# phbgomes22/FastFourierConvolution

Measured on AMD Instinct MI355X. Metric: FFC-generator fwd images/sec @ B=256 64×64×3; % HBM roofline; max |Δ| vs ref, higher is better.
Workload: dtype f32; 1 GPU; FFCGenerator(nz=100,nc=3,ngf=64) forward 64x64x3; global_batch=256, per_gpu_batch=256, bn_mode=train, spectral_mix=fp32, hipgraph=True, parallelism=dp1

## Files before the change

### fastfourierconvolution_amd/_plan.py

```python
from __future__ import annotations

from dataclasses import dataclass, field

import os

import numpy as np

CONVQ_TCMAX = int(os.environ.get("FFC_CONVQ_TCMAX", "0"))

BK = 16
MPAD = 128
TILE_CFGS = {0: (128, 128, 2), 1: (64, 128, 2), 2: (32, 256, 4)}
PAD_ENTRY = (15, 0, 0, 0)


@dataclass(frozen=True)
class Seg:
    kind: str
    C: int
    IH: int
    IW: int
    k: int = 1
    s: int = 1
    p: int = 0
# ... 202 lines not shown
    OH: int
    OW: int
    Sy: int
    Sx: int
    segs: tuple
    mults: list
    cpad: list
    org: list
    prc: list
    vec4: list
    rowlen: list
    phases: list
    ktab: np.ndarray
    taptab: np.ndarray
    a_size: int
    cfg: int
    NS: int
    TR: int
    TC: int
    nrb: int
    ncb: int
    cc: list = field(default_factory=list)
    q: bool = False
    mt: int = 1
    direct: list = field(default_factory=list)
    qstride: list = field(default_factory=list)
    ksplit: int = 1

    @property
    def Mpad(self):
        return -(-self.M // MPAD) * MPAD

    @property
    def npb(self):
        return -(-self.B // self.NS) * self.nrb * self.ncb


PATCH_MAX_UNITS = 8 * 256


def patch_units_per_row(PC: int, vec4: bool, aligned: bool = False) -> int:
    if not vec4:
        return PC
    return -(-PC // 4) if aligned else (PC + 6) // 4


def plan_patch_job(B: int, M: int, segs, cfg: int | None = None):
    segs = tuple(segs)
    if any(sg.pool or sg.gate for sg in segs):
        return None
    base = plan_job(B, M, segs)
    NP = base.Sy * base.Sx
    if NP not in (1, 4) or len(base.phases) != NP:
        return None
    if cfg is None:
        cfg = 0 if NP == 4 else 2
    np_, ntw = PATCH_CFGS[cfg]
    if np_ != NP:
        return None
    npix = (4 // NP) * ntw * 32
    PHm = max(ph.PH for ph in base.phases)
    PWm = max(ph.PW for ph in base.phases)
    TC = min(PWm, npix)
    TR = min(PHm, max(1, npix // TC))
    NS = max(1, min(B, npix // (TR * TC)))
    nrb, ncb = -(-PHm // TR), -(-PWm // TC)
    taps = []
    cc = [PATCH_CC] * len(segs)
    for ph in base.phases:
        row = []
        for si, sg in enumerate(segs):
            ty = _taps(sg, base.Sy, ph.py, sg.IH, ph.PH)
            tx = _taps(sg, base.Sx, ph.px, sg.IW, ph.PW)
            if NP == 1 and len(ty) == len(tx) == 3 and (sg.kind == "conv" or (sg.kind == "convT" and sg.s == 1)):
                ty, tx = sorted(ty, key=lambda t: t[1]), sorted(tx, key=lambda t: t[1])
                if any(b[1] - a[1] != 1 for a, b in zip(ty, ty[1:])) or any(b[1] - a[1] != 1 for a, b in zip(tx, tx[1:])):
                    return None
                ty = ty + [(-1, ty[-1][1] + 1)]
                tx = tx + [(-1, tx[-1][1] + 1)]
            T = len(ty) * len(tx)
            if T == 16 and NP == 1 and len(ty) == len(tx) == 4:
                cc[si] = 4
            elif T and 4 % T:
                return None
            row.append((ty, tx))
        taps.append(row)
    cpad = [-(-sg.C // cc[si]) * cc[si] for si, sg in enumerate(segs)]
    org, prc, vec4, rowlen = [], [], [], []
    for si, sg in enumerate(segs):
        oys = [o for row in taps for (k, o) in row[si][0]]
        oxs = [o for row in taps for (k, o) in row[si][1]]
        if not oys or not oxs:
            oys, oxs = [0], [0]
        my_, mx_ = base.mults[si]
        oy0, ox0 = min(oys), min(oxs)
        PR = (TR - 1) * my_ + (max(oys) - oy0) + 1
        PC = (TC - 1) * mx_ + (max(oxs) - ox0) + 1
        v4 = sg.IW % 4 == 0
        al = ox0 % 4 == 0 and (TC * mx_) % 4 == 0
        if NS * cc[si] * PR * patch_units_per_row(PC, v4, al) > PATCH_MAX_UNITS:
            return None
        vec4.append(v4)
        rowlen.append(4 * patch_units_per_row(PC, True, al) if v4 else PC)
        org.append((oy0, ox0))
        prc.append((PR, PC))
    phases, ktab, taptab = [], [], []
    a_total = 0
    Mpad = -(-M // MPAD) * MPAD
    for pi, ph in enumerate(base.phases):
        d = dict(py=ph.py, px=ph.px, PH=ph.PH, PW=ph.PW, T=[], kseg=[], tap_base=[], tap_h=[])
        k = 0
        kt_off = len(ktab)
        for si, sg in enumerate(segs):
            ty, tx = taps[pi][si]
            T = len(ty) * len(tx)
            d["T"].append(T)
            d["kseg"].append(k)
            d["tap_base"].append(len(taptab))
            PR, PC = prc[si]
            base_t = len(taptab)
            for (ky, oy) in ty:
                for (kx, ox) in tx:
                    taptab.append(((oy - org[si][0]) << 16) | (ox - org[si][1]))
            th = 0
            if T == 16:
                dyx = [(t >> 16, t & 0xFFFF) for t in taptab[base_t:]]
                hy, hx = dyx[8][0] - dyx[0][0], dyx[8][1] - dyx[0][1]
                if hx < 0 or any((dyx[j + 8][0] - dyx[j][0], dyx[j + 8][1] - dyx[j][1]) != (hy, hx)
                                 for j in range(8)):
                    return None
                th = (hy << 16) | hx
            d["tap_h"].append(th)
            for ch in range(cpad[si]):
                for (ky, oy) in ty:
                    for (kx, ox) in tx:
                        ktab.append((si | (ch << 4), oy, ox, ky | (kx << 16))
                                    if ch < sg.C and ky >= 0 and kx >= 0 else PAD_ENTRY)
            k += cpad[si] * T
        if k == 0:
            return None
        d["Kpad"] = k
        d["K"] = k
        d["kt_off"] = kt_off
        d["a_off"] = a_total
        a_total += Mpad * k
        phases.append(d)
    return PatchPlan(B, M, base.OH, base.OW, base.Sy, base.Sx, segs, base.mults, cpad, org, prc, vec4, rowlen, phases,
                     np.asarray(ktab, dtype=np.int32).reshape(-1, 4), np.asarray(taptab or [0], dtype=np.int32),
                     a_total, cfg, NS, TR, TC, nrb, ncb, cc)


CONVQ_CFGS = {0: (1, 4), 1: (1, 2), 2: (2, 2), 3: (1, 1)}
CONVQ_MAX_UNITS = 256
CONVQ_LDS_BUDGET = 150 * 1024


def convq_strides(NS, TR, TC, PR, PC, pad=True):
    if not pad:
        return PC, PR * PC
    qr = PC + ((TC - PC) % 16)
    qs = PR * qr + ((TR * TC - PR * qr) % 16)
    return qr, qs


def convq_lds_bytes(NS, strides):
    return 3 * (((max(NS * qs for _, qs in strides) * 96 + 255) // 256) * 256 + 256)


def plan_convq_job(B: int, M: int, segs, cfg: int):
    segs = tuple(segs)
    if any(sg.pool or sg.gate for sg in segs):
        return None
    base = plan_job(B, M, segs)
    if (base.Sy, base.Sx) != (2, 2) or len(base.phases) != 4:
        return None
    mt, ntw = CONVQ_CFGS[cfg]
    npix = 32 * ntw
    PHm = max(ph.PH for ph in base.phases)
    PWm = max(ph.PW for ph in base.phases)
    TC = min(PWm, npix)
    if CONVQ_TCMAX >= 4 and TC > CONVQ_TCMAX:
        TC = CONVQ_TCMAX
    TR = min(PHm, max(1, npix // TC))
    NS = max(1, min(B, npix // (TR * TC)))
    nrb, ncb = -(-PHm // TR), -(-PWm // TC)
    direct = [sg.kind == "pw" for sg in segs]
    taps = []
    for ph in base.phases:
        row = []
        for si, sg in enumerate(segs):
            ty = _taps(sg, base.Sy, ph.py, sg.IH, ph.PH)
            tx = _taps(sg, base.Sx, ph.px, sg.IW, ph.PW)
            T = len(ty) * len(tx)
            if (direct[si] and T not in (0, 1)) or T > 4:
                return None
            row.append((ty, tx))
        taps.append(row)
    cpad = [-(-sg.C // 16) * 16 for sg in segs]
    org, prc = [], []
    for si, sg in enumerate(segs):
        my_, mx_ = base.mults[si]
        if direct[si]:
            if (my_, mx_) != (2, 2):
                return None
            org.append((0, 0))
            prc.append((1, 1))
            continue
        oys = [o for row in taps for (k, o) in row[si][0]] or [0]
        oxs = [o for row in taps for (k, o) in row[si][1]] or [0]
        oy0, ox0 = min(oys), min(oxs)
        PR = (TR - 1) * my_ + (max(oys) - oy0) + 1
        PC = (TC - 1) * mx_ + (max(oxs) - ox0) + 1
        if sg.IW % 4:
            return None
        PC = 4 * patch_units_per_row(PC, True, False)
        if 2 * NS * PR * (PC // 4) > CONVQ_MAX_UNITS:
            return None
        org.append((oy0, ox0))
        prc.append((PR, PC))
    staged = [prc[si] for si in range(len(segs)) if not direct[si]]
    pad = bool(staged) and convq_lds_bytes(NS, [convq_strides(NS, TR, TC, PR, PC) for PR, PC in staged]) \
        <= CONVQ_LDS_BUDGET
    if os.environ.get("FFC_CONVQ_PAD") == "0":
        pad = False
    qstride = [convq_strides(NS, TR, TC, PR, PC, pad) for (PR, PC) in prc]
    if staged and convq_lds_bytes(NS, [qstride[si] for si in range(len(segs)) if not direct[si]]) > 160 * 1024:
        return None
    if any(not direct[si] and B * sg.C * sg.IH * sg.IW * 4 >= 0x7FFFFFFF for si, sg in enumerate(segs)):
        return None
    phases, ktab, taptab = [], [], []
    a_total = 0
    Mpad = -(-M // MPAD) * MPAD
    for pi, ph in enumerate(base.phases):
        d = dict(py=ph.py, px=ph.px, PH=ph.PH, PW=ph.PW, T=[], kseg=[], tap_base=[], tap_h=[])
        k = 0
        kt_off = len(ktab)
        for si, sg in enumerate(segs):
            ty, tx = taps[pi][si]
            T = len(ty) * len(tx)
            d["T"].append(T)
            d["kseg"].append(k)
            d["tap_base"].append(len(taptab))
            d["tap_h"].append(0)
            tl = [(ky, oy, kx, ox) for (ky, oy) in ty for (kx, ox) in tx]
            TT = 1 if direct[si] else 4
            d["T"][-1] = TT
            for t in range(TT):
                taptab.append(((tl[t][1] - org[si][0]) << 16) | (tl[t][3] - org[si][1]) if t < T else 0)
            for c0 in range(0, cpad[si], 16):
                for t in range(TT):
                    for ch in range(c0, c0 + 16):
                        if t < T and ch < sg.C:
                            ky, oy, kx, ox = tl[t]
                            ktab.append((si | (ch << 4), oy, ox, ky | (kx << 16)))
                        else:
                            ktab.append(PAD_ENTRY)
            k += cpad[si] * TT
        if k == 0:
            return None
        d["Kpad"] = k
        d["K"] = k
        d["kt_off"] = kt_off
        d["a_off"] = a_total
        a_total += Mpad * k
        phases.append(d)
    return PatchPlan(B, M, base.OH, base.OW, base.Sy, base.Sx, segs, base.mults, cpad, org, prc,
                     [not d for d in direct], [pc for (_, pc) in prc], phases,
                     np.asarray(ktab, dtype=np.int32).reshape(-1, 4), np.asarray(taptab or [0], dtype=np.int32),
                     a_total, cfg, NS, TR, TC, nrb, ncb, [16] * len(segs), True, mt, direct, qstride)


CONVQ_SPLIT_FIXED = 17500.0


def convq_chunks(q) -> int:
    return sum(c // 16 for c in q.cpad)


def convq_cost(q, ksplit: int = 1) -> float:
    wgs = q.npb * (-(-q.M // (32 * q.mt))) * ksplit
    mt, ntw = CONVQ_CFGS[q.cfg]
    slots = 256 * (2 if (mt, ntw) == (1, 1) else 1)
    per_wg = -(-convq_chunks(q) // ksplit) * (768.0 * mt * ntw + 5500.0)
    return -(-wgs // slots) * (per_wg + (CONVQ_SPLIT_FIXED if ksplit > 1 else 0.0))


_TUNED = None


def job_signature(B, M, segs) -> tuple:
    return (int(B), int(M), tuple((sg.kind, sg.C, sg.IH, sg.IW, sg.k, sg.s, sg.p, sg.d, sg.op, sg.pool, sg.gate)
                                  for sg in segs))


def convq_tuned():
    global _TUNED
    if _TUNED is None:
        import json
        jobs, groups = {}, {}
        path = os.environ.get("FFC_CONVQ_TUNED", os.path.join(os.path.dirname(os.path.abspath(__file__)),
                                                               "convq_tuned.json"))
        if path and os.path.exists(path):
            with open(path) as f:
                for e in json.load(f)["entries"]:
                    sigs = tuple(sorted((B, M, tuple(tuple(sg) for sg in segs)) for B, M, segs in e["jobs"]))
                    groups[sigs] = (int(e["cfg"]), int(e["ksplit"]))
                    for sg in sigs:
                        jobs[sg] = int(e["cfg"])
        _TUNED = (jobs, groups)
    return _TUNED


def pick_convq_ksplit(q) -> int:
    return pick_convq_ksplit_group([q])


def pick_convq_ksplit_group(plans) -> int:
    cmin = min(convq_chunks(q) for q in plans)
    force = os.environ.get("FFC_CONVQ_KSPLIT")
    if force is not None:
        return max(1, min(8, int(force), cmin))
    tuned = convq_tuned()[1].get(tuple(sorted(job_signature(q.B, q.M, q.segs) for q in plans)))
    if tuned is not None and tuned[0] == plans[0].cfg:
        return max(1, min(tuned[1], cmin))
    ks = [k for k in (1, 2, 4, 8) if k == 1 or cmin >= 4 * k]
    return min(ks, key=lambda k: (sum(convq_cost(q, k) for q in plans), k))


def convq_slot_tiles(tiles) -> np.ndarray:
    first = tiles[(tiles[:, 3] & 7) == 0]
    out = np.zeros((first.shape[0], 4), dtype=np.int32)
    out[first[:, 3] >> 3, :3] = first[:, :3]
    return out


def pick_convq_cfg(B, M, segs):
    force = os.environ.get("FFC_CONVQ_CFG")
    tuned = convq_tuned()[0].get(job_signature(B, M, segs))
    if os.environ.get("FFC_CONVQ_TUNED_LOG"):
        import sys
        print(f"[convq] tuned cfg {'hit' if tuned is not None else 'miss'}: {job_signature(B, M, segs)}",
              file=sys.stderr)
    if force is not None:
        cands = [int(force)]
    elif tuned is not None:
        cands = [tuned]
    else:
        cands = ([0, 2] if M >= 64 else [0]) + [1, 3]
    plans = [q for q in (plan_convq_job(B, M, segs, c) for c in cands) if q is not None]
    for q in plans:
        q.ksplit = pick_convq_ksplit(q)
    return min(plans, key=lambda q: convq_cost(q, q.ksplit)) if plans else None


def pick_patch_cfg(B, M, segs, min_blocks=512):
    force = os.environ.get("FFC_PATCH_CFG4")
    if force is not None:
        q = plan_patch_job(B, M, segs, int(force))
        if q is not None:
            return q
    p = plan_patch_job(B, M, segs)
    if p is None:
        return plan_patch_job(B, M, segs, 1) or plan_patch_job(B, M, segs, 3)
    if p.cfg == 0:
        blocks = p.npb * (-(-M // 32))
        if blocks < min_blocks:
            q = plan_patch_job(B, M, segs, 1)
            if q is not None:
                return q
# ... 32 lines not shown
```

### fastfourierconvolution_amd/csrc/convq_kernels.hip

```cpp
#include "ffc_internal.h"

#include <algorithm>
#include <cstdlib>
#include <map>
#include <mutex>
#include <string>
#include <tuple>

namespace {

constexpr int QTHREADS = 512;
#ifndef FFC_CONVQ_WPE
#define FFC_CONVQ_WPE
#endif
#ifndef FFC_CONVQ_SLOTS
#define FFC_CONVQ_SLOTS 2
#endif
constexpr int QSLOTS = FFC_CONVQ_SLOTS;
static_assert(QSLOTS >= 2 && QSLOTS <= 6, "convq staging slots");

struct ConvQArgs {
    ffc_convp_job jobs[2];
    const int4* tiles;
    int ebuf;
// ... 119 lines not shown
        if (cl == 0 && m < E.M) stp[m] = make_float4(cnt, mean, m2, 0.0f);
    }
}

template <int MT, int NTW>
__device__ __forceinline__ void convq_epilogue(const ffc_convp_job& J, int wave, int lane, int pb, int m0,
                                               floatx16 (&acc)[MT][NTW]) {
    const QGeom<NTW> g = q_geometry<NTW>(J, wave, lane, pb);
    const ffc_convp_phase& P = J.ph[wave];
    const QEpi E = q_epi(J);
    const int py = P.py, px = P.px;
    const int h = lane >> 5, cl = lane & 31;
    const size_t plane = (size_t)E.OH * E.OW;
    long long obase[NTW];
#pragma unroll
    for (int nt = 0; nt < NTW; ++nt)
        obase[nt] = (long long)(g.b0 + g.pns[nt]) * E.M * (long long)plane +
                    ((g.r0 + g.pr_[nt]) * 2 + py) * E.OW + ((g.c0 + g.pc_[nt]) * 2 + px);
    bool allv = m0 + 32 * MT <= E.M;
#pragma unroll
    for (int nt = 0; nt < NTW; ++nt) allv = allv && g.pv[nt];
    const bool full = __builtin_amdgcn_ballot_w64(allv) == ~0ull;
    unsigned voff[NTW];
#pragma unroll
    for (int nt = 0; nt < NTW; ++nt) {
        voff[nt] = ((unsigned)g.pns[nt] * (unsigned)E.M * (unsigned)plane + (unsigned)(4 * h) * (unsigned)plane +
                    (unsigned)(((g.r0 + g.pr_[nt]) * 2 + py) * E.OW + ((g.c0 + g.pc_[nt]) * 2 + px))) * 4u;
        asm volatile("" : "+v"(voff[nt]));
    }
#pragma unroll
    for (int mt = 0; mt < MT; ++mt) {
        floatx16 (&tacc)[NTW] = acc[mt];
        const int mbase = m0 + 32 * mt + 4 * h;
        if (E.bias || E.addend) {
#pragma unroll
            for (int r = 0; r < 16; ++r) {
                const int m = mbase + (r & 3) + 8 * (r >> 2);
                if (m >= E.M) continue;
                const float bv = E.bias ? E.bias[m] : 0.0f;
#pragma unroll
                for (int nt = 0; nt < NTW; ++nt) {
                    float v = tacc[nt][r] + bv;
                    if (E.addend && g.pv[nt]) v += E.addend[obase[nt] + (long long)m * plane];
                    tacc[nt][r] = v;
                }
            }
        }
        if (E.stats) q_stats<NTW>(E, wave, cl, pb, mbase, g.pv, tacc);
        if (full) {
#pragma unroll
            for (int r = 0; r < 16; ++r) {
                float* sb = E.out + ((size_t)g.b0 * E.M + m0 + 32 * mt + (r & 3) + 8 * (r >> 2)) * plane;
#pragma unroll
                for (int nt = 0; nt < NTW; ++nt) {
                    *reinterpret_cast<float*>(reinterpret_cast<char*>(sb) + voff[nt]) = q_act(tacc[nt][r], E.slope);
                }
            }
            continue;
        }
#pragma unroll
        for (int r = 0; r < 16; ++r) {
            const int m = mbase + (r & 3) + 8 * (r >> 2);
            if (m < E.M) {
#pragma unroll
                for (int nt = 0; nt < NTW; ++nt)
                    if (g.pv[nt]) E.out[obase[nt] + (long long)m * plane] = q_act(tacc[nt][r], E.slope);
            }
        }
    }
}

typedef float floatx2 __attribute__((ext_vector_type(2)));
template <int PX>
struct StageVec {
    float v[PX];
};
template <int PX>
__device__ __forceinline__ StageVec<PX> stage_ld(__amdgpu_buffer_rsrc_t rs, int voff, int soff) {
    StageVec<PX> r;
    if constexpr (PX == 4) {
        const floatx4 q = __builtin_bit_cast(floatx4, __builtin_amdgcn_raw_buffer_load_b128(rs, voff, soff, 0));
        r.v[0] = q[0]; r.v[1] = q[1]; r.v[2] = q[2]; r.v[3] = q[3];
    } else if constexpr (PX == 2) {
        const floatx2 q = __builtin_bit_cast(floatx2, __builtin_amdgcn_raw_buffer_load_b64(rs, voff, soff, 0));
        r.v[0] = q[0]; r.v[1] = q[1];
    } else {
        r.v[0] = __builtin_bit_cast(float, __builtin_amdgcn_raw_buffer_load_b32(rs, voff, soff, 0));
    }
    return r;
}

template <int MT, int NTW, int SL = QSLOTS, int PX = 4>
__device__ __forceinline__ void convq_tile(const ConvQArgs& args, const int tix, char* lds) {
    static_assert(SL >= 2 && SL <= 6, "convq staging slots");
    static_assert(PX == 1 || PX == 2 || PX == 4, "pixels per staging unit");
    const int tid = threadIdx.x, lane = tid & 63;
    const int wave_id = __builtin_amdgcn_readfirstlane(tid >> 6);
    const bool stager = wave_id >= 4;
    const int wave = wave_id & 3;
    const int stid = tid - 256;
    const int h = lane >> 5, cl = lane & 31;
    const int4 tile = args.tiles[tix];
    const int ji = __builtin_amdgcn_readfirstlane(tile.x);
    const int m0 = __builtin_amdgcn_readfirstlane(tile.y);
    const int pb = __builtin_amdgcn_readfirstlane(tile.z);
    const int tw = __builtin_amdgcn_readfirstlane(tile.w);
    const int ks = tw & 7, slot = tw >> 3;
    const int nsplit = args.ksplit;
    const ffc_convp_job& J = args.jobs[ji];
    const ffc_convp_phase& P = J.ph[wave];
    const int ebuf = args.ebuf;

    const int NS = J.NS, TR = J.TR, TC = J.TC;
    const int bs = pb / (J.nrb * J.ncb);
    const int prem = pb - bs * J.nrb * J.ncb;
    const int rb = prem / J.ncb, cb = prem - rb * J.ncb;
    const int b0 = bs * NS, r0 = rb * TR, c0 = cb * TC;
    const int TRC = TR * TC;
    const int nseg = J.nseg;


    floatx16 acc[MT][NTW];
#pragma unroll
    for (int mt = 0; mt < MT; ++mt)
#pragma unroll
        for (int nt = 0; nt < NTW; ++nt)
#pragma unroll
            for (int r = 0; r < 16; ++r) acc[mt][nt][r] = 0.0f;

#ifdef FFC_TRACE_Q
    const unsigned long long tq_rt0 = __builtin_amdgcn_s_memrealtime();
    unsigned long long tq_0, tq_a, tq_b, tq_c, tq_d, tq_bar = 0, tq_A = 0, tq_mf = 0;
    QSTAMP(tq_0);
#endif
    const int ksteps = P.Kpad >> 4;
    const uint16_t* __restrict__ Afrag = J.A3 + 3 * P.a_off + (size_t)(m0 >> 5) * ksteps * 1536 + lane * 8;
    auto load_A = [&](int k, Split3 (&a)[MT]) {
#pragma unroll
        for (int mt = 0; mt < MT; ++mt) {
            const uint16_t* f = Afrag + ((size_t)mt * ksteps + (k >> 4)) * 1536;
            a[mt].hi = __builtin_bit_cast(bf16x8, *reinterpret_cast<const u32x4*>(f));
            a[mt].mid = __builtin_bit_cast(bf16x8, *reinterpret_cast<const u32x4*>(f + 512));
            a[mt].lo = __builtin_bit_cast(bf16x8, *reinterpret_cast<const u32x4*>(f + 1024));
        }
    };

    struct {
        __amdgpu_buffer_rsrc_t rs;
        unsigned voff;
        unsigned cstride;
        int C, Cpad, cfull;
        int hu8;
        int wb;
    } st;
    auto stage_setup = [&](int s) {
        const ffc_convp_seg& S = J.seg[s];
        const int IHW = S.IH * S.IW;
        st.rs = ffc::buf_rsrc(S.x, (unsigned long long)J.B * S.C * IHW * 4);
        st.C = S.C;
        st.Cpad = S.Cpad;
        st.cfull = (S.C & 15) == 0;
        st.cstride = (unsigned)IHW * 4u;
        const int PR = S.PR, G = S.PC / PX, QR = S.qrow, QS = S.qsample;
        const int ngrp = NS * PR * G;
        const int nunits = 2 * ngrp;
        const int iy0 = r0 * S.mult_y + S.org_y;
        const int xa = (c0 * S.mult_x + S.org_x) & ~3;
        const int n = stid;
        const int hu = n >= ngrp ? 1 : 0;
        const int q = n - hu * ngrp;
        const int g = q % G, q1 = q / G;
        const int pr = q1 % PR, ns = q1 / PR;
        const int b = b0 + ns, iy = iy0 + pr, ix = xa + PX * g;
        const bool ok = n < nunits && b < J.B && (unsigned)iy < (unsigned)S.IH && (unsigned)ix < (unsigned)S.IW;
        st.voff = ok ? (unsigned)(((b * S.C + 8 * hu) * IHW + iy * S.IW + ix) * 4) : ffc::OOB;
        st.hu8 = 8 * hu;
        st.wb = n < nunits ? ((hu * NS + ns) * QS + pr * QR + PX * g) * 48 : -1;
    };
    auto stage_load = [&](StageVec<PX> (&sv)[8], int ch0) {
        const unsigned sbase = (unsigned)ch0 * st.cstride;
#pragma unroll
        for (int j = 0; j < 8; ++j) {
            const unsigned vo = (st.cfull || ch0 + st.hu8 + j < st.C) ? st.voff : ffc::OOB;
            sv[j] = stage_ld<PX>(st.rs, (int)vo, (int)(sbase + (unsigned)j * st.cstride));
        }
    };
    auto stage_store = [&](const StageVec<PX> (&sv)[8], int wb, char* buf) {
        if (wb >= 0) {
#pragma unroll
            for (int e = 0; e < PX; ++e) {
                float v8[8];
#pragma unroll
                for (int j = 0; j < 8; ++j) v8[j] = sv[j].v[e];
                const Split3 sp = split3(v8);
                u32x4* d = reinterpret_cast<u32x4*>(buf + wb + 48 * e);
                d[0] = __builtin_bit_cast(u32x4, sp.hi);
                d[1] = __builtin_bit_cast(u32x4, sp.mid);
                d[2] = __builtin_bit_cast(u32x4, sp.lo);
            }
        }
    };

    int kseg = 0, cpad = 0;
    int fb[NTW];
    int tb[4];
    auto geom = [&](int s, int (&fbo)[NTW], int (&tbo)[4]) {
        const ffc_convp_seg& S = J.seg[s];
        const QGeom<NTW> g = q_geometry<NTW>(J, wave, lane, pb);
        const int QR = S.qrow, QS = S.qsample, nimg = NS * QS;
        const int ix0 = c0 * S.mult_x + S.org_x, xoff = ix0 - (ix0 & ~3);
#pragma unroll
        for (int nt = 0; nt < NTW; ++nt)
            fbo[nt] = (h * nimg + g.pns[nt] * QS + g.pr_[nt] * S.mult_y * QR + g.pc_[nt] * S.mult_x + xoff) * 48;
#pragma unroll
        for (int t = 0; t < 4; ++t) {
            const int tt = P.tap[s][t];
            tbo[t] = ((tt >> 16) * QR + (tt & 0xFFFF)) * 48;
        }
    };
    auto compute_setup = [&](int s) {
        kseg = P.kseg[s];
        cpad = J.seg[s].Cpad;
        geom(s, fb, tb);
    };

    int nstaged = 0, ndirect = 0;
    for (int s = 0; s < nseg; ++s) {
        if (J.seg[s].direct) ndirect += J.seg[s].Cpad >> 4;
        else nstaged += J.seg[s].Cpad >> 4;
    }
    const int ntot = nstaged + ndirect;
    const int lo = ntot * ks / nsplit, hi = ntot * (ks + 1) / nsplit;
    const int slo = min(lo, nstaged), nst = min(hi, nstaged) - slo;
    const int dlo = max(lo, nstaged) - nstaged, dhi = max(hi, nstaged) - nstaged;

    const int npad = (nst + SL - 1) / SL * SL;
    if (nst > 0) {
        int ss = 0;
        while (J.seg[ss].direct) ++ss;
        int c0k = slo;
        while (c0k >= (J.seg[ss].Cpad >> 4)) {
            c0k -= J.seg[ss].Cpad >> 4;
            do { ++ss; } while (J.seg[ss].direct);
        }
        int cs = ss, sch = 16 * c0k, cch = 16 * c0k;
        if (stager) {
#ifdef FFC_TRACE_Q
            unsigned long long q0, qa, qb, ql = 0, qs = 0, qw = 0, qi = 0;
            QSTAMP(q0);
#endif
            StageVec<PX> sv[SL][8];
            int wbs[SL];
            stage_setup(ss);
            int ic = 0;
            auto issue = [&](StageVec<PX> (&dst)[8], int& wb) {
                const bool live = ss < nseg && ic < nst;
                ++ic;
                stage_load(dst, live ? sch : 0);
                wb = live ? st.wb : -1;
                if (live) {
                    sch += 16;
                    if (sch >= st.Cpad) {
                        do { ++ss; } while (ss < nseg && J.seg[ss].direct);
                        sch = 0;
                        if (ss < nseg) stage_setup(ss);
                    }
                }
            };
            auto store_timed = [&](const StageVec<PX> (&src)[8], int wb, char* buf) {
#ifdef FFC_TRACE_Q
                QSTAMP(qa);
                float chk = src[0].v[0] + src[7].v[PX - 1];
                asm volatile("" ::"v"(chk));
                QSTAMP(qb);
                ql += qb - qa;
                stage_store(src, wb, buf);
                QSTAMP(qa);
                qs += qa - qb;
#else
                stage_store(src, wb, buf);
#endif
            };
            auto bar = [&]() {
#ifdef FFC_TRACE_Q
                QSTAMP(qa);
#endif
#ifndef FFC_QPROBE_NOBAR
                __syncthreads();
#endif
#ifdef FFC_TRACE_Q
                QSTAMP(qb);
                qw += qb - qa;
#endif
            };
#pragma unroll
            for (int u = 0; u < SL; ++u) issue(sv[u], wbs[u]);
            store_timed(sv[0], wbs[0], lds);
            issue(sv[0], wbs[0]);
            store_timed(sv[1 % SL], wbs[1 % SL], lds + ebuf);
            bar();
            int wbuf = 2;
            for (int c0 = 1; c0 <= npad; c0 += SL) {
#pragma unroll
                for (int u = 0; u < SL; ++u) {
#ifndef FFC_QPROBE_NOSTAGE
#ifdef FFC_TRACE_Q
                    QSTAMP(qa);
#endif
                    issue(sv[(1 + u) % SL], wbs[(1 + u) % SL]);
#ifdef FFC_TRACE_Q
                    QSTAMP(qb);
                    qi += qb - qa;
#endif
                    store_timed(sv[(2 + u) % SL], wbs[(2 + u) % SL], lds + wbuf * ebuf);
#endif
                    wbuf = wbuf == 2 ? 0 : wbuf + 1;
                    bar();
                }
            }
#ifdef FFC_TRACE_Q
            QSTAMP(qa);
            if (tid == 256) {
                unsigned long long* tr = g_ffc_trace_q + 16 * tix;
                tr[9] = ql;
                tr[10] = qs;
                tr[11] = qw;
                tr[12] = qa - q0;
                tr[13] = nst;
                tr[14] = qi;
            }
#endif
            return;
        }
        Split3 a[4][MT];
        compute_setup(cs);
        int pf[NTW];
#pragma unroll
        for (int nt = 0; nt < NTW; ++nt) pf[nt] = fb[nt] + tb[0];
#pragma unroll
        for (int t = 0; t < 4; ++t) load_A(kseg + cch * 4 + 16 * t, a[t]);
        u32x4 bq[2][NTW][3];
        auto read_frag = [&](const char* base, const int (&off)[NTW], int add, u32x4 (&dst)[NTW][3]) {
#pragma unroll
            for (int nt = 0; nt < NTW; ++nt) {
                const char* p1 = base + off[nt] + add;
                dst[nt][0] = lds_read16(p1, 0);
                dst[nt][1] = lds_read16(p1, 16);
                dst[nt][2] = lds_read16(p1, 32);
            }
        };
#ifdef FFC_TRACE_Q
        QSTAMP(tq_a);
#endif
        __syncthreads();
#ifdef FFC_TRACE_Q
        QSTAMP(tq_b);
        tq_bar += tq_b - tq_a;
#endif
        read_frag(lds, pf, 0, bq[0]);
        int rbuf = 0;
        for (int ci = 0; ci < nst; ++ci) {
#ifdef FFC_TRACE_Q
            QSTAMP(tq_a);
#endif
            const bool more = ci + 1 < nst;
            const int nbuf = rbuf == 2 ? 0 : rbuf + 1;
            const char* cur = lds + rbuf * ebuf;
            const char* nxt = lds + nbuf * ebuf;
            int cn = cs, chn = cch + 16;
            const bool segchg = more && chn >= cpad;
            int kn;
            if (segchg) {
                do { ++cn; } while (J.seg[cn].direct);
                chn = 0;
                kn = P.kseg[cn];
                int fbn[NTW], tbn[4];
                geom(cn, fbn, tbn);
#pragma unroll
                for (int nt = 0; nt < NTW; ++nt) pf[nt] = fbn[nt] + tbn[0];
            } else {
                kn = kseg + (more ? chn : cch) * 4;
            }
            __builtin_amdgcn_sched_barrier(0);
#ifdef FFC_TRACE_Q
            QSTAMP(tq_b);
            tq_A += tq_b - tq_a;
#endif
#ifndef FFC_QPROBE_NOMFMA
#pragma unroll
            for (int t = 0; t < 4; ++t) {
                if (t + 1 < 4) read_frag(cur, fb, tb[t + 1], bq[(t + 1) & 1]);
                else read_frag(nxt, pf, 0, bq[0]);
#pragma unroll
                for (int nt = 0; nt < NTW; ++nt) {
                    Split3 b;
                    b.hi = __builtin_bit_cast(bf16x8, bq[t & 1][nt][0]);
                    b.mid = __builtin_bit_cast(bf16x8, bq[t & 1][nt][1]);
                    b.lo = __builtin_bit_cast(bf16x8, bq[t & 1][nt][2]);
#pragma unroll
                    for (int mt = 0; mt < MT; ++mt) acc[mt][nt] = mfma_split3(a[t][mt], b, acc[mt][nt]);
                }
#ifndef FFC_QPROBE_NOA
                load_A(kn + 16 * t, a[t]);
#endif
                __builtin_amdgcn_sched_group_barrier(0x100, 3 * NTW, 0);
                __builtin_amdgcn_sched_group_barrier(0x8, 6 * NTW * MT, 0);
                __builtin_amdgcn_sched_group_barrier(0x20, 3 * MT, 0);
                __builtin_amdgcn_sched_barrier(0);
            }
#endif
#ifdef FFC_TRACE_Q
            QSTAMP(tq_a);
            tq_mf += tq_a - tq_b;
#endif
            if (segchg) {
                cs = cn;
                cch = 0;
                compute_setup(cs);
            } else {
                cch += 16;
            }
            rbuf = nbuf;
#ifdef FFC_TRACE_Q
            QSTAMP(tq_a);
#endif
#ifndef FFC_QPROBE_NOBAR
            __syncthreads();
#endif
#ifdef FFC_TRACE_Q
            QSTAMP(tq_b);
            tq_bar += tq_b - tq_a;
#endif
        }
#ifndef FFC_QPROBE_NOBAR
        for (int ci = nst; ci < npad; ++ci) __syncthreads();
#endif
    }
#ifdef FFC_TRACE_Q
    QSTAMP(tq_c);
#endif
    if (stager) return;

    int dbase = 0;
    for (int s = 0; s < nseg; ++s) {
        const ffc_convp_seg& S = J.seg[s];
        if (!S.direct) continue;
        const int nch = S.Cpad >> 4;
        const int c_lo = max(dlo - dbase, 0), c_hi = min(dhi - dbase, nch);
        dbase += nch;
        if (c_lo >= c_hi) continue;
        const int IHW = S.IH * S.IW;
        const QGeom<NTW> g = q_geometry<NTW>(J, wave, lane, pb);
        const bool* pv = g.pv;
        const float* xp[NTW];
#pragma unroll
        for (int nt = 0; nt < NTW; ++nt) {
            const int oy = (r0 + g.pr_[nt]) * J.Sy + P.py, ox = (c0 + g.pc_[nt]) * J.Sx + P.px;
            const int b = pv[nt] ? b0 + g.pns[nt] : 0;
            xp[nt] = S.x + ((long long)b * S.C + 8 * h) * IHW + (pv[nt] ? oy * S.IW + ox : 0);
        }
        for (int ch0 = 16 * c_lo; ch0 < 16 * c_hi; ch0 += 16) {
            Split3 a[MT];
            load_A(P.kseg[s] + ch0, a);
            float bv[NTW][8];
#pragma unroll
            for (int nt = 0; nt < NTW; ++nt)
#pragma unroll
// ... 3 lines not shown
                    bv[nt][j] = ok ? v : 0.0f;
                }
#pragma unroll
            for (int nt = 0; nt < NTW; ++nt) {
                const Split3 b = split3(bv[nt]);
#pragma unroll
                for (int mt = 0; mt < MT; ++mt) acc[mt][nt] = mfma_split3(a[mt], b, acc[mt][nt]);
            }
        }
    }

#ifdef FFC_QPROBE_NOEPI
    if (acc[0][0][0] != 1234.5f) return;
#endif
    if (nsplit > 1) {
        store_partial<MT, NTW>(args.part + ((size_t)(slot * nsplit + ks) * 4 + wave) * (MT * NTW * 1024), lane, acc);
        return;
    }
#ifdef FFC_TRACE_Q
    QSTAMP(tq_d);
#endif
    convq_epilogue<MT, NTW>(J, wave, lane, pb, m0, acc);
#ifdef FFC_TRACE_Q
    {
        unsigned long long tq_e;
        QSTAMP(tq_e);
        if (tid == 0) {
            unsigned long long* tr = g_ffc_trace_q + 16 * tix;
            tr[0] = tq_rt0;
            tr[1] = __builtin_amdgcn_s_memrealtime();
            tr[2] = (unsigned long long)__builtin_amdgcn_s_getreg((31 << 11) | 4) |
                    ((unsigned long long)__builtin_amdgcn_s_getreg((31 << 11) | 20) << 32);
            tr[3] = tq_bar;
            tr[4] = tq_A;
            tr[5] = tq_mf;
            tr[6] = tq_d - tq_c;
            tr[7] = tq_e - tq_d;
            tr[8] = tq_e - tq_0;
        }
    }
#endif
}

template <int MT, int NTW, int SL = QSLOTS, int PX = 4>
__global__ __launch_bounds__(QTHREADS) FFC_CONVQ_WPE void convq_kernel(ConvQArgs args_byval) {
#if defined(__HIP_DEVICE_COMPILE__)
    const ConvQArgs& args = *(const ConvQArgs*)__builtin_amdgcn_kernarg_segment_ptr();
#else
    const ConvQArgs& args = args_byval;
#endif
    extern __shared__ __attribute__((aligned(16))) char lds[];
    for (int tix = blockIdx.x; tix < args.ntiles; tix += gridDim.x) convq_tile<MT, NTW, SL, PX>(args, tix, lds);
}

template <int MT, int NTW>
__global__ __launch_bounds__(256) void convq_reduce_kernel(ConvQArgs args_byval, const int4* __restrict__ slots) {
#if defined(__HIP_DEVICE_COMPILE__)
    const ConvQArgs& args = *(const ConvQArgs*)__builtin_amdgcn_kernarg_segment_ptr();
#else
    const ConvQArgs& args = args_byval;
#endif
    const int lane = threadIdx.x & 63;
    const int wave = __builtin_amdgcn_readfirstlane(threadIdx.x >> 6);
    const int4 tile = slots[blockIdx.x];
    const int ji = __builtin_amdgcn_readfirstlane(tile.x);
    const int m0 = __builtin_amdgcn_readfirstlane(tile.y);
    const int pb = __builtin_amdgcn_readfirstlane(tile.z);
    const int nsplit = args.ksplit;
    constexpr int FR = MT * NTW * 1024;
    const float* base = args.part + ((size_t)blockIdx.x * nsplit * 4 + wave) * FR + lane * 4;
    floatx16 acc[MT][NTW];
#pragma unroll
    for (int mt = 0; mt < MT; ++mt)
#pragma unroll
        for (int nt = 0; nt < NTW; ++nt)
#pragma unroll
            for (int r4 = 0; r4 < 4; ++r4) {
                const float* p = base + ((mt * NTW + nt) * 4 + r4) * 256;
                floatx4 v[8];
#pragma unroll
                for (int k = 0; k < 8; ++k)
                    v[k] = *reinterpret_cast<const floatx4*>(p + (size_t)(k < nsplit ? k : 0) * 4 * FR);
                floatx4 sum = v[0];
#pragma unroll
                for (int k = 1; k < 8; ++k)
                    if (k < nsplit) sum += v[k];
#pragma unroll
                for (int e = 0; e < 4; ++e) acc[mt][nt][4 * r4 + e] = sum[e];
            }
    convq_epilogue<MT, NTW>(args.jobs[ji], wave, lane, pb, m0, acc);
}

int persistent_grid(const void* k, size_t lds, int ntiles) {
    static const bool off = [] {
        const char* e = getenv("FFC_CONVQ_PERSIST");
        return e && e[0] == '0';
    }();
    if (off) return ntiles;
    static std::mutex mu;
    static std::map<std::tuple<const void*, size_t, int>, int> cache;
    int dev = 0;
    if (hipGetDevice(&dev) != hipSuccess) {
        ffc::set_error("ffc_convq_forward: hipGetDevice failed");
        return -1;
    }
    int slots = 0;
    {
        std::lock_guard<std::mutex> g(mu);
        auto it = cache.find({k, lds, dev});
        if (it != cache.end()) {
            slots = it->second;
        } else {
            int cus = 0, per = 0;
            if (hipDeviceGetAttribute(&cus, hipDeviceAttributeMultiprocessorCount, dev) != hipSuccess ||
                hipOccupancyMaxActiveBlocksPerMultiprocessor(&per, k, QTHREADS, lds) != hipSuccess || cus <= 0) {
                ffc::set_error("ffc_convq_forward: occupancy query failed");
                return -1;
            }
            slots = cus * (per > 0 ? per : 1);
            slots = slots >= 8 ? slots / 8 * 8 : slots;
            cache[{k, lds, dev}] = slots;
        }
    }
    return ntiles < slots ? ntiles : slots;
}

template <int MT, int NTW, int SL = QSLOTS, int PX = 4>
int launch_q(const ConvQArgs& a, int ntiles, size_t lds, hipStream_t s, const int4* slots, int nslots) {
    auto k = convq_kernel<MT, NTW, SL, PX>;
    if (lds > 64 * 1024) {
        static bool raised = false;
        if (!raised) {
            const hipError_t e = hipFuncSetAttribute(reinterpret_cast<const void*>(k),
                                                     hipFuncAttributeMaxDynamicSharedMemorySize, 160 * 1024);
            if (e != hipSuccess) {
                ffc::set_error(std::string("ffc_convq_forward: hipFuncSetAttribute: ") + hipGetErrorString(e));
                return FFC_E_LAUNCH;
            }
            raised = true;
        }
    }
    const int grid = persistent_grid(reinterpret_cast<const void*>(k), lds, ntiles);
    if (grid <= 0) return FFC_E_LAUNCH;
    hipLaunchKernelGGL(k, dim3(grid), dim3(QTHREADS), lds, s, a);
    if (a.ksplit > 1) {
        const int rc = ffc::launch_status("ffc_convq_forward_split");
        if (rc != FFC_OK) return rc;
        auto r = convq_reduce_kernel<MT, NTW>;
        hipLaunchKernelGGL(r, dim3(nslots), dim3(256), 0, s, a, slots);
    }
    return ffc::launch_status("ffc_convq_forward_split");
}

int stage_px(int units4) {
    static const int force = [] {
        const char* e = getenv("FFC_CONVQ_PX");
        return e ? atoi(e) : 0;
    }();
    const int fit = 4 * units4 <= 256 ? 1 : (2 * units4 <= 256 ? 2 : 4);
    return (force == 1 || force == 2 || force == 4) && force >= fit ? force : fit;
}

int slots11() {
    static const int v = [] {
        const char* e = getenv("FFC_CONVQ_SLOTS11");
        const int n = e ? atoi(e) : 0;
        return (n == 3 || n == 4) ? n : QSLOTS;
    }();
    return v;
}

}

namespace {
__global__ void q_act_inplace_kernel(float* __restrict__ x, long long n, int act) {
    for (long long i = (long long)blockIdx.x * blockDim.x + threadIdx.x; i < n; i += (long long)gridDim.x * blockDim.x) {
        const float v = x[i];
        float y;
        switch (act) {
            case FFC_ACT_TANH: y = tanhf(v); break;
            case FFC_ACT_SIGMOID: y = 1.0f / (1.0f + expf(-v)); break;
            default: y = 0.5f * v * (1.0f + erff(v * 0.70710678118654752f)); break;
        }
        x[i] = y;
    }
}

__global__ void pack_a3_kernel(const float* __restrict__ A, ffc_convp_job J, uint16_t* __restrict__ A3, long long total) {
    for (long long i = (long long)blockIdx.x * blockDim.x + threadIdx.x; i < total; i += (long long)gridDim.x * blockDim.x) {
        long long r = i;
        int p = 0;
        long long nfr = 0;
        for (; p < J.nphase; ++p) {
            nfr = (long long)(J.Mpad >> 5) * (J.ph[p].Kpad >> 4) * 64;
            if (r < nfr) break;
            r -= nfr;
        }
        const int lane = (int)(r & 63);
        const long long fr = r >> 6;
        const int ks = J.ph[p].Kpad >> 4;
        const int mtile = (int)(fr / ks), kstep = (int)(fr - (long long)mtile * ks);
        const int m = 32 * mtile + (lane & 31), k0 = 16 * kstep + 8 * (lane >> 5);
        const float* src = A + J.ph[p].a_off + (size_t)m * J.ph[p].Kpad + k0;
        float v[8];
#pragma unroll
        for (int j = 0; j < 8; ++j) v[j] = src[j];
        const Split3 sp = split3(v);
        uint16_t* dst = A3 + 3 * J.ph[p].a_off + (fr * 3) * 512 + lane * 8;
        *reinterpret_cast<u32x4*>(dst) = __builtin_bit_cast(u32x4, sp.hi);
        *reinterpret_cast<u32x4*>(dst + 512) = __builtin_bit_cast(u32x4, sp.mid);
        *reinterpret_cast<u32x4*>(dst + 1024) = __builtin_bit_cast(u32x4, sp.lo);
    }
}
}

extern "C" int ffc_convq_pack_a3(const ffc_convp_job* job, const float* A, uint16_t* A3, void* stream) {
    FFC_CHECK_ARG(job && A && A3 && job->nphase >= 1 && job->nphase <= 4 && job->Mpad % 32 == 0,
                  "ffc_convq_pack_a3: bad args");
    FFC_CHECK_ARG((reinterpret_cast<uintptr_t>(A3) & 15) == 0, "ffc_convq_pack_a3: A3 must be 16-byte aligned");
    long long total = 0;
    for (int p = 0; p < job->nphase; ++p) {
        FFC_CHECK_ARG(job->ph[p].Kpad % 16 == 0 && job->ph[p].Kpad > 0, "ffc_convq_pack_a3: Kpad % 16");
        total += (long long)(job->Mpad >> 5) * (job->ph[p].Kpad >> 4) * 64;
    }
    const long long blocks = (total + 255) / 256;
    hipLaunchKernelGGL(pack_a3_kernel, dim3((unsigned)(blocks < 4096 ? blocks : 4096)), dim3(256), 0,
                       (hipStream_t)stream, A, *job, A3, total);
    return ffc::launch_status("ffc_convq_pack_a3");
}

#ifdef FFC_TRACE_Q
extern "C" int ffc_debug_trace_read_q(void* dst, size_t bytes) {
    return hipMemcpyFromSymbol(dst, HIP_SYMBOL(g_ffc_trace_q), bytes, 0, hipMemcpyDeviceToHost) == hipSuccess ? 0 : -1;
}
#endif

extern "C" int ffc_convq_config(int cfg, int* mt, int* ntw) {
    static const int T[4][2] = {{1, 4}, {1, 2}, {2, 2}, {1, 1}};
    if (cfg < 0 || cfg > 3 || !mt || !ntw) return FFC_E_INVALID;
    *mt = T[cfg][0];
    *ntw = T[cfg][1];
    return FFC_OK;
}

extern "C" long long ffc_convq_split_floats(int cfg, int nslots, int ksplit) {
    int MT = 0, NTW = 0;
    if (ffc_convq_config(cfg, &MT, &NTW) != FFC_OK || nslots < 0 || ksplit < 1 || ksplit > 8) return -1;
    return ksplit > 1 ? (long long)nslots * ksplit * 4 * MT * NTW * 1024 : 0;
}

extern "C" int ffc_convq_forward(const ffc_convp_job* jobs, int njobs, const int* tiles, int ntiles, int cfg,
                                 void* stream) {
    return ffc_convq_forward_split(jobs, njobs, tiles, ntiles, nullptr, 0, cfg, 1, nullptr, stream);
}

extern "C" int ffc_convq_forward_split(const ffc_convp_job* jobs, int njobs, const int* tiles, int ntiles,
                                       const int* slot_tiles, int nslots, int cfg, int ksplit, float* part,
                                       void* stream) {
    FFC_CHECK_ARG(jobs && tiles && njobs >= 1 && njobs <= 2 && ntiles > 0, "ffc_convq_forward: bad args");
    int MT = 0, NTW = 0;
    FFC_CHECK_ARG(ffc_convq_config(cfg, &MT, &NTW) == FFC_OK, "ffc_convq_forward: unknown cfg");
    FFC_CHECK_ARG(ksplit >= 1 && ksplit <= 8, "ffc_convq_forward: 1 <= ksplit <= 8");
    FFC_CHECK_ARG(ksplit == 1 || (part && (reinterpret_cast<uintptr_t>(part) & 15) == 0),
                  "ffc_convq_forward: ksplit > 1 needs the partial buffer (16-byte aligned)");
    FFC_CHECK_ARG(ksplit == 1 || (slot_tiles && nslots > 0 && (long long)nslots * ksplit == ntiles),
                  "ffc_convq_forward: ksplit > 1 needs the slot table (ntiles = nslots * ksplit)");
    int npix_max = 0, units4 = 0;
    for (int j = 0; j < njobs; ++j) {
        const ffc_convp_job& J = jobs[j];
        FFC_CHECK_ARG(J.A3 && J.out && J.B > 0 && J.M > 0, "ffc_convq_forward: incomplete job (needs the A3 planes)");
        FFC_CHECK_ARG((reinterpret_cast<uintptr_t>(J.A3) & 15) == 0 && J.a3_stride % 8 == 0,
                      "ffc_convq_forward: A3 planes need 16-byte alignment");
        FFC_CHECK_ARG(J.nphase == 4 && J.Sy == 2 && J.Sx == 2, "ffc_convq_forward: 4-phase (stride-2) jobs only");
        FFC_CHECK_ARG(J.nseg >= 1 && J.nseg <= FFC_MAX_SEG, "ffc_convq_forward: nseg out of range");
        FFC_CHECK_ARG(J.Mpad % 128 == 0 && J.Mpad >= J.M, "ffc_convq_forward: Mpad");
        FFC_CHECK_ARG((unsigned long long)J.NS * J.M * J.OH * J.OW * 4 < 0xFFFFFFFFull,
                      "ffc_convq_forward: a pixel block's output span must fit 32-bit offsets");
        FFC_CHECK_ARG(J.NS > 0 && J.TR > 0 && J.TC > 0 && J.nrb > 0 && J.ncb > 0 && J.NS * J.TR * J.TC <= 32 * NTW,
                      "ffc_convq_forward: pixel block");
        for (int p = 0; p < 4; ++p) FFC_CHECK_ARG(J.ph[p].Kpad % 16 == 0, "ffc_convq_forward: Kpad % 16");
        for (int s = 0; s < J.nseg; ++s) {
            const ffc_convp_seg& S = J.seg[s];
            FFC_CHECK_ARG(S.x && S.Cpad % 16 == 0 && S.Cpad >= S.C && S.cc == 16, "ffc_convq_forward: segment channels");
            FFC_CHECK_ARG(!S.pool && !S.gate, "ffc_convq_forward: pooled / gated segments use ffc_conv_forward");
            for (int p = 0; p < 4; ++p) {
                const int T = J.ph[p].T[s];
                FFC_CHECK_ARG(S.direct ? T == 1 : T == 4,
                              "ffc_convq_forward: taps per phase (4 staged, 1 direct; the plan pads)");
            }
            if (S.direct) {
                FFC_CHECK_ARG(S.mult_y == 2 && S.mult_x == 2 && S.IH == J.OH && S.IW == J.OW,
                              "ffc_convq_forward: direct segments are 1x1 at the output resolution");
            } else {
                FFC_CHECK_ARG(S.PR > 0 && S.PC > 0 && S.PC % 4 == 0 && S.qrow >= S.PC && S.qsample >= S.PR * S.qrow,
                              "ffc_convq_forward: patch shape / LDS strides");
                FFC_CHECK_ARG(S.vec4 && S.IW % 4 == 0 && (reinterpret_cast<uintptr_t>(S.x) & 15) == 0,
                              "ffc_convq_forward: staged segments need IW % 4 == 0 and a 16-byte aligned input");
                FFC_CHECK_ARG((unsigned long long)J.B * S.C * S.IH * S.IW * 4 < 0x7FFFFFFFull,
                              "ffc_convq_forward: staged segments are read through 32-bit buffer offsets (< 2 GiB)");
                FFC_CHECK_ARG(2 * J.NS * S.PR * (S.PC / 4) <= 256,
                              "ffc_convq_forward: patch too large for the staging waves (one unit per thread)");
                if (2 * J.NS * S.PR * (S.PC / 4) > units4) units4 = 2 * J.NS * S.PR * (S.PC / 4);
                const int npix = J.NS * S.qsample;
                if (npix > npix_max) npix_max = npix;
            }
        }
    }
    const size_t ebuf = ((size_t)npix_max * 96 + 255) / 256 * 256 + 256;
    size_t lds = npix_max > 0 ? 3 * ebuf : 16;
    FFC_CHECK_ARG(lds <= 160 * 1024, "ffc_convq_forward: patch too large");
    ConvQArgs a;
    a.ebuf = (int)ebuf;
    a.jobs[0] = jobs[0];
    a.jobs[1] = jobs[njobs > 1 ? 1 : 0];
    a.tiles = reinterpret_cast<const int4*>(tiles);
    a.ksplit = ksplit;
    a.part = part;
    a.ntiles = ntiles;
    const int4* sl = reinterpret_cast<const int4*>(slot_tiles);
    hipStream_t s = (hipStream_t)stream;
    bool post[2] = {false, false};
    for (int j = 0; j < 2; ++j) {
        ffc_convp_job& Jc = a.jobs[j];
        if (Jc.act == FFC_ACT_TANH || Jc.act == FFC_ACT_SIGMOID || Jc.act == FFC_ACT_GELU) {
            post[j] = j < njobs;
            Jc.act = FFC_ACT_IDENTITY;
        }
    }
    const int px = stage_px(units4);
    int rc = FFC_E_INVALID;
    switch (cfg) {
        case 0:
            if (px <= 2) rc = launch_q<1, 4, QSLOTS, 2>(a, ntiles, lds, s, sl, nslots);
            else rc = launch_q<1, 4>(a, ntiles, lds, s, sl, nslots);
            break;
        case 1:
            if (px <= 2) rc = launch_q<1, 2, QSLOTS, 2>(a, ntiles, lds, s, sl, nslots);
            else rc = launch_q<1, 2>(a, ntiles, lds, s, sl, nslots);
            break;
        case 2:
            if (px <= 2) rc = launch_q<2, 2, QSLOTS, 2>(a, ntiles, lds, s, sl, nslots);
            else rc = launch_q<2, 2>(a, ntiles, lds, s, sl, nslots);
            break;
        case 3:
            if (slots11() == 3) rc = launch_q<1, 1, 3>(a, ntiles, lds, s, sl, nslots);
            else if (slots11() == 4) rc = launch_q<1, 1, 4>(a, ntiles, lds, s, sl, nslots);
            else if (px == 1) rc = launch_q<1, 1, QSLOTS, 1>(a, ntiles, lds, s, sl, nslots);
            else if (px == 2) rc = launch_q<1, 1, QSLOTS, 2>(a, ntiles, lds, s, sl, nslots);
            else rc = launch_q<1, 1>(a, ntiles, lds, s, sl, nslots);
            break;
        default: ffc::set_error("ffc_convq_forward: unknown cfg"); return FFC_E_INVALID;
    }
    if (rc != FFC_OK) return rc;
    for (int j = 0; j < njobs; ++j) {
        if (!post[j]) continue;
        const long long n = (long long)jobs[j].B * jobs[j].M * jobs[j].OH * jobs[j].OW;
        const long long blocks = (n + 255) / 256;
        hipLaunchKernelGGL(q_act_inplace_kernel, dim3((unsigned)(blocks < 8192 ? blocks : 8192)), dim3(256), 0, s,
                           jobs[j].out, n, jobs[j].act);
        rc = ffc::launch_status("ffc_convq_forward (activation pass)");
        if (rc != FFC_OK) return rc;
    }
    return FFC_OK;
}
```

Measured before the change: 596,400 images/s.

## Stage only in-image patch units and zero halo LDS entries separately

The staging threads in the convq kernel now map only to patch units that fall inside the image. Out-of-image halo slots are zero-filled directly in LDS, on the first few stages of each segment only. Because the thread-count limit now applies to in-image units rather than the full padded patch, larger tiles or fewer stage_px splits qualify, and staging work on edge tiles shrinks. Index decomposition uses float reciprocals instead of integer division, which adds a small risk of rounding error in the index maths and some extra setup work.

```diff
diff --git a/fastfourierconvolution_amd/_plan.py b/fastfourierconvolution_amd/_plan.py
--- a/fastfourierconvolution_amd/_plan.py
+++ b/fastfourierconvolution_amd/_plan.py
@@ -378,6 +378,7 @@
 
 CONVQ_CFGS = {0: (1, 4), 1: (1, 2), 2: (2, 2), 3: (1, 1)}
 CONVQ_MAX_UNITS = 256
+CONVQ_MAX_PATCH_UNITS = 512
 CONVQ_LDS_BUDGET = 150 * 1024
 
 
@@ -387,6 +388,13 @@
     qr = PC + ((TC - PC) % 16)
     qs = PR * qr + ((TR * TC - PR * qr) % 16)
     return qr, qs
+
+
+def convq_inimage_units(B, NS, TR, TC, nrb, ncb, mult, org, PR, PC, IH, IW):
+    nr = max(min(PR, IH - iy0) - max(-iy0, 0) for iy0 in (rb * TR * mult[0] + org[0] for rb in range(nrb)))
+    ng = max(min(PC // 4, (IW - xa) // 4) - max(-xa, 0) // 4
+             for xa in ((cb * TC * mult[1] + org[1]) & ~3 for cb in range(ncb)))
+    return 2 * min(NS, B) * nr * ng
 
 
 def convq_lds_bytes(NS, strides):
@@ -440,7 +448,8 @@
         if sg.IW % 4:
             return None
         PC = 4 * patch_units_per_row(PC, True, False)
-        if 2 * NS * PR * (PC // 4) > CONVQ_MAX_UNITS:
+        if convq_inimage_units(B, NS, TR, TC, nrb, ncb, (my_, mx_), (oy0, ox0), PR, PC, sg.IH, sg.IW) \
+                > CONVQ_MAX_UNITS or 2 * NS * PR * (PC // 4) > CONVQ_MAX_PATCH_UNITS:
             return None
         org.append((oy0, ox0))
         prc.append((PR, PC))
diff --git a/fastfourierconvolution_amd/csrc/convq_kernels.hip b/fastfourierconvolution_amd/csrc/convq_kernels.hip
--- a/fastfourierconvolution_amd/csrc/convq_kernels.hip
+++ b/fastfourierconvolution_amd/csrc/convq_kernels.hip
@@ -295,6 +295,7 @@
         int C, Cpad, cfull;
         int hu8;
         int wb;
+        int zb[2];
     } st;
     auto stage_setup = [&](int s) {
         const ffc_convp_seg& S = J.seg[s];
@@ -305,20 +306,47 @@
         st.cfull = (S.C & 15) == 0;
         st.cstride = (unsigned)IHW * 4u;
         const int PR = S.PR, G = S.PC / PX, QR = S.qrow, QS = S.qsample;
-        const int ngrp = NS * PR * G;
-        const int nunits = 2 * ngrp;
         const int iy0 = r0 * S.mult_y + S.org_y;
         const int xa = (c0 * S.mult_x + S.org_x) & ~3;
+        const int nsv = min(NS, J.B - b0);
+        const int pr_lo = max(-iy0, 0), nr = min(PR, S.IH - iy0) - pr_lo;
+        const int g_lo = max(-xa, 0) / PX, ng = min(G, (S.IW - xa) / PX) - g_lo;
+        const int ngrp = (nr > 0 && ng > 0) ? nsv * nr * ng : 0;
+        const int nunits = 2 * ngrp;
+        const int nrd = max(nr, 1), ngd = max(ng, 1);
         const int n = stid;
         const int hu = n >= ngrp ? 1 : 0;
         const int q = n - hu * ngrp;
-        const int g = q % G, q1 = q / G;
-        const int pr = q1 % PR, ns = q1 / PR;
+        const int q1 = (int)(((float)q + 0.5f) * __builtin_amdgcn_rcpf((float)ngd)), g = g_lo + q - q1 * ngd;
+        const int ns = (int)(((float)q1 + 0.5f) * __builtin_amdgcn_rcpf((float)nrd)), pr = pr_lo + q1 - ns * nrd;
         const int b = b0 + ns, iy = iy0 + pr, ix = xa + PX * g;
-        const bool ok = n < nunits && b < J.B && (unsigned)iy < (unsigned)S.IH && (unsigned)ix < (unsigned)S.IW;
+        const bool ok = n < nunits;
         st.voff = ok ? (unsigned)(((b * S.C + 8 * hu) * IHW + iy * S.IW + ix) * 4) : ffc::OOB;
         st.hu8 = 8 * hu;
-        st.wb = n < nunits ? ((hu * NS + ns) * QS + pr * QR + PX * g) * 48 : -1;
+        st.wb = ok ? ((hu * NS + ns) * QS + pr * QR + PX * g) * 48 : -1;
+        const int npg = NS * PR * G;
+        const float rG = __builtin_amdgcn_rcpf((float)G), rPR = __builtin_amdgcn_rcpf((float)PR);
+#pragma unroll
+        for (int k = 0; k < 2; ++k) {
+            const int m = stid + 256 * k;
+            const int zh = m >= npg ? 1 : 0;
+            const int zq = m - zh * npg;
+            const int zq1 = (int)(((float)zq + 0.5f) * rG), zg = zq - zq1 * G;
+            const int zns = (int)(((float)zq1 + 0.5f) * rPR), zpr = zq1 - zns * PR;
+            const bool in = b0 + zns < J.B && (unsigned)(iy0 + zpr) < (unsigned)S.IH &&
+                            (unsigned)(xa + PX * zg) < (unsigned)S.IW;
+            st.zb[k] = (m < 2 * npg && !in) ? ((zh * NS + zns) * QS + zpr * QR + PX * zg) * 48 : -1;
+        }
+    };
+    auto zero_halo = [&](const int (&zb)[2], char* buf) {
+        const u32x4 z = {0u, 0u, 0u, 0u};
+#pragma unroll
+        for (int k = 0; k < 2; ++k)
+            if (zb[k] >= 0) {
+                u32x4* d = reinterpret_cast<u32x4*>(buf + zb[k]);
+#pragma unroll
+                for (int i = 0; i < 3 * PX; ++i) d[i] = z;
+            }
     };
     auto stage_load = [&](StageVec<PX> (&sv)[8], int ch0) {
         const unsigned sbase = (unsigned)ch0 * st.cstride;
@@ -394,23 +422,30 @@
 #endif
             StageVec<PX> sv[SL][8];
             int wbs[SL];
+            int zbs[SL][2];
+            int zc = 0;
             stage_setup(ss);
             int ic = 0;
-            auto issue = [&](StageVec<PX> (&dst)[8], int& wb) {
+            auto issue = [&](StageVec<PX> (&dst)[8], int& wb, int (&zb)[2]) {
                 const bool live = ss < nseg && ic < nst;
                 ++ic;
                 stage_load(dst, live ? sch : 0);
                 wb = live ? st.wb : -1;
+                zb[0] = live && zc < 3 ? st.zb[0] : -1;
+                zb[1] = live && zc < 3 ? st.zb[1] : -1;
                 if (live) {
+                    ++zc;
                     sch += 16;
                     if (sch >= st.Cpad) {
                         do { ++ss; } while (ss < nseg && J.seg[ss].direct);
                         sch = 0;
+                        zc = 0;
                         if (ss < nseg) stage_setup(ss);
                     }
                 }
             };
-            auto store_timed = [&](const StageVec<PX> (&src)[8], int wb, char* buf) {
+            auto store_timed = [&](const StageVec<PX> (&src)[8], int wb, const int (&zb)[2], char* buf) {
+                zero_halo(zb, buf);
 #ifdef FFC_TRACE_Q
                 QSTAMP(qa);
                 float chk = src[0].v[0] + src[7].v[PX - 1];
@@ -437,10 +472,10 @@
 #endif
             };
 #pragma unroll
-            for (int u = 0; u < SL; ++u) issue(sv[u], wbs[u]);
-            store_timed(sv[0], wbs[0], lds);
-            issue(sv[0], wbs[0]);
-            store_timed(sv[1 % SL], wbs[1 % SL], lds + ebuf);
+            for (int u = 0; u < SL; ++u) issue(sv[u], wbs[u], zbs[u]);
+            store_timed(sv[0], wbs[0], zbs[0], lds);
+            issue(sv[0], wbs[0], zbs[0]);
+            store_timed(sv[1 % SL], wbs[1 % SL], zbs[1 % SL], lds + ebuf);
             bar();
             int wbuf = 2;
             for (int c0 = 1; c0 <= npad; c0 += SL) {
@@ -450,12 +485,12 @@
 #ifdef FFC_TRACE_Q
                     QSTAMP(qa);
 #endif
-                    issue(sv[(1 + u) % SL], wbs[(1 + u) % SL]);
+                    issue(sv[(1 + u) % SL], wbs[(1 + u) % SL], zbs[(1 + u) % SL]);
 #ifdef FFC_TRACE_Q
                     QSTAMP(qb);
                     qi += qb - qa;
 #endif
-                    store_timed(sv[(2 + u) % SL], wbs[(2 + u) % SL], lds + wbuf * ebuf);
+                    store_timed(sv[(2 + u) % SL], wbs[(2 + u) % SL], zbs[(2 + u) % SL], lds + wbuf * ebuf);
 #endif
                     wbuf = wbuf == 2 ? 0 : wbuf + 1;
                     bar();
@@ -765,12 +800,25 @@
     return ffc::launch_status("ffc_convq_forward_split");
 }
 
-int stage_px(int units4) {
+int inimage_units4(const ffc_convp_job& J, const ffc_convp_seg& S) {
+    int nr = 0, ng = 0;
+    for (int rb = 0; rb < J.nrb; ++rb) {
+        const int iy0 = rb * J.TR * S.mult_y + S.org_y;
+        nr = std::max(nr, std::min(S.PR, S.IH - iy0) - std::max(-iy0, 0));
+    }
+    for (int cb = 0; cb < J.ncb; ++cb) {
+        const int xa = (cb * J.TC * S.mult_x + S.org_x) & ~3;
+        ng = std::max(ng, std::min(S.PC / 4, (S.IW - xa) / 4) - std::max(-xa, 0) / 4);
+    }
+    return 2 * std::min(J.NS, J.B) * nr * ng;
+}
+
+int stage_px(int units4, int patch4) {
     static const int force = [] {
         const char* e = getenv("FFC_CONVQ_PX");
         return e ? atoi(e) : 0;
     }();
-    const int fit = 4 * units4 <= 256 ? 1 : (2 * units4 <= 256 ? 2 : 4);
+    const int fit = 4 * units4 <= 256 && 4 * patch4 <= 512 ? 1 : (2 * units4 <= 256 && 2 * patch4 <= 512 ? 2 : 4);
     return (force == 1 || force == 2 || force == 4) && force >= fit ? force : fit;
 }
 
@@ -878,7 +926,7 @@
                   "ffc_convq_forward: ksplit > 1 needs the partial buffer (16-byte aligned)");
     FFC_CHECK_ARG(ksplit == 1 || (slot_tiles && nslots > 0 && (long long)nslots * ksplit == ntiles),
                   "ffc_convq_forward: ksplit > 1 needs the slot table (ntiles = nslots * ksplit)");
-    int npix_max = 0, units4 = 0;
+    int npix_max = 0, units4 = 0, patch4 = 0;
     for (int j = 0; j < njobs; ++j) {
         const ffc_convp_job& J = jobs[j];
         FFC_CHECK_ARG(J.A3 && J.out && J.B > 0 && J.M > 0, "ffc_convq_forward: incomplete job (needs the A3 planes)");
@@ -911,9 +959,13 @@
                               "ffc_convq_forward: staged segments need IW % 4 == 0 and a 16-byte aligned input");
                 FFC_CHECK_ARG((unsigned long long)J.B * S.C * S.IH * S.IW * 4 < 0x7FFFFFFFull,
                               "ffc_convq_forward: staged segments are read through 32-bit buffer offsets (< 2 GiB)");
-                FFC_CHECK_ARG(2 * J.NS * S.PR * (S.PC / 4) <= 256,
-                              "ffc_convq_forward: patch too large for the staging waves (one unit per thread)");
-                if (2 * J.NS * S.PR * (S.PC / 4) > units4) units4 = 2 * J.NS * S.PR * (S.PC / 4);
+                const int u4 = inimage_units4(J, S);
+                FFC_CHECK_ARG(u4 <= 256,
+                              "ffc_convq_forward: patch too large for the staging waves (one in-image unit per thread)");
+                if (u4 > units4) units4 = u4;
+                const int p4 = 2 * J.NS * S.PR * (S.PC / 4);
+                FFC_CHECK_ARG(p4 <= 512, "ffc_convq_forward: patch too large for the staging waves (halo units)");
+                if (p4 > patch4) patch4 = p4;
                 const int npix = J.NS * S.qsample;
                 if (npix > npix_max) npix_max = npix;
             }
@@ -940,7 +992,7 @@
             Jc.act = FFC_ACT_IDENTITY;
         }
     }
-    const int px = stage_px(units4);
+    const int px = stage_px(units4, patch4);
     int rc = FFC_E_INVALID;
     switch (cfg) {
         case 0:
```

Result: no change. 598,400 images/s, median of 4 (+0.3%).
